# FabianPlum/SMILify

Measured on AMD Instinct MI355X. Metric: SMIL fit-iters/sec (LBS+render+loss) per GPU at 1/2/4/8 MI355X, higher is better.
Workload: dtype f32

## Files before the change

smilify_amd/csrc/raster.hip:

```cpp
#include "common.h"

#define TILE 8
#define DCHUNK 32
#define FREC 28
#define FSTR 28
#define K_EPS 1e-8f
#define ALPHA_GRAD_EPS 1e-12f
#ifndef SEL_BITS
#define SEL_BITS 5
#endif
#ifndef SEL1_BITS
#define SEL1_BITS 6
#endif
#define SAT8 160u
#ifndef DGROUP
#define DGROUP 4
#endif
#ifndef KGROUP
#define KGROUP 4
#endif
#ifndef SELR
#define SELR 6
#endif
#ifndef REC_CAP
#define REC_CAP 65536
#endif
#define REC_PAD 64
#ifndef RESIDENT_PER_CU
#define RESIDENT_PER_CU 16
#endif

#ifndef WAVES_PER_SIMD
#define WAVES_PER_SIMD 4
#endif
enum { MODE_FWD = 0, MODE_BWD = 1, MODE_FUSED = 2 };

#include "raster_hooks.h"

#define N_CLASSES 4
#ifndef PACKED_MIN_IMAGES
#define PACKED_MIN_IMAGES 64
#endif
#ifndef CLASS_T0
#define CLASS_T0 65536
#endif
#define CLASS_T1 16384
#define CLASS_T2 4096
#ifndef SPLIT0_LOG
#define SPLIT0_LOG 0
#endif
#define COUNT_TILES_MAX 4096
#define N_PARTS 8
struct RasterCounters {
    unsigned int n_class[N_PARTS][N_CLASSES];
    struct { unsigned int next, pad[15]; } deal[N_PARTS];
    unsigned int straddling;
    unsigned int unclipped;
    unsigned int tie_pixels;
    unsigned int tie_next;
};

__host__ __device__ __forceinline__ unsigned int deal_split_log(unsigned int n_items, unsigned int slots) {
    return n_items * 8u <= slots * 5u / 8u ? 3u : (n_items * 4u <= slots * 5u / 4u ? 2u : (n_items * 2u <= slots * 5u / 4u ? 1u : 0u));
}
__host__ __device__ __forceinline__ unsigned int deal_working(unsigned int n_items, unsigned int split_log, unsigned int slots) {
    const unsigned int w = (n_items << split_log) * 7u / 16u;
    return w > slots / 8u ? w : slots / 8u;
}

struct Rec3 { uint32_t a, b, c; };
struct TriIds { int a, b, c; };

#define CLIP_CUTS 1024
#define CLIP_FX (2 * CLIP_CUTS)
#define CLIP_VX (2 * CLIP_CUTS)
struct ClipTables {
    float *xv;
    int *xf;
    int2 *xsrc;
    float2 *xcoef;
    float *xg;
    uint32_t *xcount;
    int *xparent;
};
__host__ __device__ __forceinline__ int faces_padded(int F) { return (F + WAVE - 1) / WAVE * WAVE; }
__device__ __forceinline__ int face_vertex(const int *__restrict__ faces, const int *__restrict__ xf_n, int F, int f, int k) {
    return f < F ? faces[3 * f + k] : xf_n[3 * (f - faces_padded(F)) + k];
}
__device__ __forceinline__ const float *vertex_ptr(const float *__restrict__ vn, const float *__restrict__ xv_n, int V, int i) {
    return i < V ? vn + 3 * i : xv_n + 3 * (i - V);
}

struct RasterArgs {
    const float *verts_ndc;
    const int *faces;
    const uint32_t *tbox;
    const uint32_t *gbox;
    const uint4 *items;
    uint32_t item_cap;
    const float2 *fzr;
    RasterCounters *ctr;
    int N, V, F, S, tiles_x, K;
    int FT;
    ClipTables clip;
    float blur, sqrt_blur, inv_sigma, inv_sigma_log2e;
    float *sil;
    const float *grad_sil;
    const float *target;
    const uint8_t *target_u8;
    const float *pix_scale;
    const float *img_bound;
    int packed;
    float *loss_img;
    unsigned long long *loss_acc;
    float *d_ndc;
    const uint2 *lists;
    uint32_t list_cap;
    uint2 *slist;
    uint32_t *slist2;
    uint32_t *scfirst;
    float2 *sxy;
    TriIds *sid;
    Rec3 *srec;
    Rec3 *crec;
    int list_stride, n_cf;
    unsigned int slots;
    SmilClipDepth cd;
    int image0;
    int tie_rule;
    unsigned long long *tie_mask;
    HOOK_ARGS_FIELDS
};

__device__ __forceinline__ float pix_to_ndc(int i, int S) { return -1.0f + (2.0f * (float)i + 1.0f) / (float)S; }

__device__ __forceinline__ float edge_fn(float px, float py, float ax, float ay, float bx, float by) {
    return (px - ax) * (by - ay) - (py - ay) * (bx - ax);
}

__device__ __forceinline__ float image_fx_scale(float img_bound, float pix_scale, float inv_sigma) {
    const float bound = img_bound * fabsf(pix_scale) * sqrtf(inv_sigma);
    return (bound > 0.f && bound < 3.0e38f) ? exp2f(fminf(29.0f - floorf(log2f(bound)), 100.0f)) : 0.f;
}

template <typename T>
__device__ __forceinline__ uint32_t byte_offset(uint32_t i) {
    if (sizeof(T) == 12) {
        uint32_t r;
        asm("v_mul_u32_u24 %0, %1, 12" : "=v"(r) : "v"(i));
        return r;
    }
    return i * (uint32_t)sizeof(T);
}
template <typename T>
__device__ __forceinline__ T &at(T *base, uint32_t i) {
    i = HOOK_WRAP_IDX(i);
    return *reinterpret_cast<T *>(reinterpret_cast<char *>(base) + byte_offset<T>(i));
}
template <typename T>
__device__ __forceinline__ const T &at(const T *base, uint32_t i) {
    i = HOOK_WRAP_IDX(i);
    return *reinterpret_cast<const T *>(reinterpret_cast<const char *>(base) + byte_offset<T>(i));
}

__device__ __forceinline__ int wave_scan_add(int x) {
#define SCAN_STEP(ctrl, rows) { x += __builtin_amdgcn_update_dpp(0, x, ctrl, rows, 0xF, false); }
    SCAN_STEP(0x111, 0xF) SCAN_STEP(0x112, 0xF) SCAN_STEP(0x114, 0xF) SCAN_STEP(0x118, 0xF)
    SCAN_STEP(0x142, 0xA) SCAN_STEP(0x143, 0xC)
#undef SCAN_STEP
    return x;
}

#ifndef SETUP_THREADS
#define SETUP_THREADS 1024
#endif
// ... 697 lines not shown
    for (int i_ = lane; i_ < (1 << SEL_BITS) / 2 * WAVE; i_ += WAVE) lds.hist[i_] = 0u;
    __syncthreads();
    auto load_keys = [&](uint32_t (&kk)[KGROUP], uint32_t (&mt)[KGROUP], int g0) {
#pragma unroll
        for (int u = 0; u < KGROUP; ++u) {
            const uint32_t idx = (uint32_t)min(g0 + u * WAVE + lane, n_rec - 1);
            mt[u] = at(crec, idx).b;
            kk[u] = key_of(idx, mt[u]);
        }
    };
    auto count_keys = [&](const uint32_t (&kk)[KGROUP], const uint32_t (&mt)[KGROUP], int g0) {
        uint2 ps[KGROUP];
#pragma unroll
        for (int u = 0; u < KGROUP; ++u) ps[u] = lds.psel[mt[u] & 63u];
#pragma unroll
        for (int u = 0; u < KGROUP; ++u) {
            const uint32_t pxl = mt[u] & 63u;
            const bool hit = (g0 + u * WAVE + lane < n_rec) & (ps[u].y > 0u) & ((kk[u] >> nbits) == ps[u].x) & (kk[u] != 0xFFFFFFFFu);
            const uint32_t bucket = (kk[u] >> shift) & ((1u << b) - 1u);
            if (hit) atomicAdd(&lds.hist[(bucket >> 1) * WAVE + pxl], (bucket & 1u) ? 0x10000u : 1u);
        }
    };
    if (n_rec > 0) {
        uint32_t ka[KGROUP], ma[KGROUP], kb[KGROUP], mb[KGROUP];
        load_keys(ka, ma, 0);
        for (int g0 = 0; g0 < n_rec; g0 += 2 * KGROUP * WAVE) {
            load_keys(kb, mb, g0 + KGROUP * WAVE);
            count_keys(ka, ma, g0);
            load_keys(ka, ma, g0 + 2 * KGROUP * WAVE);
            count_keys(kb, mb, g0 + KGROUP * WAVE);
        }
    }
    __syncthreads();
}

__device__ __forceinline__ int refine_sweep(DenseLds &lds, Rec3 *crec, int n_rec, int nbits, int b,
                                            int lane, uint32_t pre, int need) {
    const int shift = nbits - b;
    lds.psel[lane] = make_uint2(pre, (uint32_t)need);
    for (int i_ = lane; i_ < (1 << SEL_BITS) / 2 * WAVE; i_ += WAVE) lds.hist[i_] = 0u;
    __syncthreads();
    int n_out = 0;
    struct CRec { uint32_t kk, mt; float lf; };
    auto load_recs = [&](CRec (&r)[KGROUP], int g0) {
#pragma unroll
        for (int u = 0; u < KGROUP; ++u) {
            const uint32_t idx = (uint32_t)min(g0 + u * WAVE + lane, n_rec - 1);
            const Rec3 q = at(crec, idx);
            r[u].kk = q.a; r[u].mt = q.b; r[u].lf = __uint_as_float(q.c);
        }
    };
    auto sift_recs = [&](const CRec (&r)[KGROUP], int g0) {
        uint2 ps[KGROUP];
#pragma unroll
        for (int u = 0; u < KGROUP; ++u) ps[u] = lds.psel[r[u].mt & 63u];
#pragma unroll
        for (int u = 0; u < KGROUP; ++u) {
            const uint32_t pxl = r[u].mt & 63u;
            const bool live = (g0 + u * WAVE + lane < n_rec) & (ps[u].y > 0u);
            const uint32_t top = r[u].kk >> nbits;
            const bool sure = live & (top < ps[u].x), stay = live & (top == ps[u].x);
            if (sure & (r[u].lf != 0.f)) atomicAdd(&lds.plog[pxl], (double)r[u].lf);
            const unsigned long long sm = __ballot(stay);
            const uint32_t slot = (uint32_t)n_out + __builtin_amdgcn_mbcnt_hi((uint32_t)(sm >> 32), __builtin_amdgcn_mbcnt_lo((uint32_t)sm, 0u));
            if (stay) {
                at(crec, slot) = Rec3{r[u].kk, r[u].mt, __float_as_uint(r[u].lf)};
                const uint32_t bucket = (r[u].kk >> shift) & ((1u << b) - 1u);
                atomicAdd(&lds.hist[(bucket >> 1) * WAVE + pxl], (bucket & 1u) ? 0x10000u : 1u);
            }
            n_out += __popcll(sm);
        }
    };
    if (n_rec > 0) {
        CRec ra[KGROUP], rb[KGROUP];
        load_recs(ra, 0);
        for (int g0 = 0; g0 < n_rec; g0 += 2 * KGROUP * WAVE) {
            load_recs(rb, g0 + KGROUP * WAVE);
            sift_recs(ra, g0);
            load_recs(ra, g0 + 2 * KGROUP * WAVE);
            sift_recs(rb, g0 + KGROUP * WAVE);
        }
    }
    __syncthreads();
    return n_out;
}

template <int MODE>
__global__ void __launch_bounds__(64, WAVES_PER_SIMD) k_raster_dense(RasterArgs a) {
    __shared__ DenseLds lds;
    const int lane = threadIdx.x;
    uint2 *const slist = a.slist + (size_t)blockIdx.x * a.list_stride;
    uint32_t *const slist2 = a.slist2 + (size_t)blockIdx.x * a.list_stride;
    uint32_t *const scfirst = a.scfirst + (size_t)blockIdx.x * a.n_cf;
    float2 *const sxy = a.sxy + (size_t)blockIdx.x * 3 * a.list_stride;
    TriIds *const sid = a.sid + (size_t)blockIdx.x * a.list_stride;
    const size_t rec0 = (size_t)blockIdx.x * (REC_CAP + REC_PAD);
    Rec3 *const srec = a.srec + rec0, *const crec = a.crec + rec0;
    const uint32_t lane_lo = lane < 32 ? 1u << lane : 0u, lane_hi = lane >= 32 ? 1u << (lane - 32) : 0u;
    const int K = a.K;
    const int n_tiles = a.tiles_x * a.tiles_x;
    unsigned int n_items_all = 0;
    for (int q = 0; q < N_PARTS; ++q)
        for (int c = 0; c < N_CLASSES; ++c) n_items_all += a.ctr->n_class[q][c];
    const unsigned int slots = a.slots;
    const unsigned int split_log = HOOK_SPLIT_LOG(deal_split_log(n_items_all, slots));
    if (blockIdx.x >= deal_working(n_items_all, split_log, slots)) return;
    const unsigned int split0_log = SPLIT0_LOG > split_log ? SPLIT0_LOG : split_log;
    const float fS = (float)a.S;
    unsigned int xcc;
    asm volatile("s_getreg_b32 %0, hwreg(HW_REG_XCC_ID)" : "=s"(xcc));
    xcc &= (unsigned int)(N_PARTS - 1);

    TIMERS_INIT
    for (unsigned int turn = 0; turn < N_PARTS; ++turn) {
    const unsigned int part = (xcc + turn) & (unsigned int)(N_PARTS - 1);
    const unsigned int nc0 = a.ctr->n_class[part][0], nc1 = a.ctr->n_class[part][1], nc2 = a.ctr->n_class[part][2], nc3 = a.ctr->n_class[part][3];
    const unsigned int n_items = nc0 + nc1 + nc2 + nc3;
    const unsigned int units0 = nc0 << split0_log;
    const unsigned int n_units = units0 + ((n_items - nc0) << split_log);
    const uint4 *const items = a.items + (size_t)part * 2u * a.item_cap;
    while (n_units > 0u) {
        unsigned int unit = 0;
        TSUB(0)
        if (lane == 0) unit = atomicAdd(&a.ctr->deal[part].next, 1u);
        unit = __builtin_amdgcn_readfirstlane(unit);
        if (unit >= n_units) break;
        TUNIT_START
        const bool heavy = unit < units0;
        const unsigned int sl = heavy ? split0_log : split_log, u_ = heavy ? unit : unit - units0;
        const unsigned int item = (u_ >> sl) + (heavy ? 0u : nc0);
        const int p_begin = (int)(u_ & ((1u << sl) - 1u)) * (WAVE >> sl), p_end = p_begin + (WAVE >> sl);
        const uint32_t item_at = item < nc0 ? item
                               : item < nc0 + nc1 ? a.item_cap - 1u - (item - nc0)
                               : item < nc0 + nc1 + nc2 ? a.item_cap + (item - nc0 - nc1)
                               : 2u * a.item_cap - 1u - (item - nc0 - nc1 - nc2);
        const uint4 it = items[item_at];
        const uint32_t code = it.x;
        const int n = (int)(code / (uint32_t)n_tiles), tile = (int)(code % (uint32_t)n_tiles);
        const int tx = tile % a.tiles_x, ty = tile / a.tiles_x;
        const int xo = tx * TILE + (lane & 7), yo = ty * TILE + (lane >> 3);
        const bool in_img = xo < a.S && yo < a.S;
        const float cx = pix_to_ndc(a.S - 1 - (tx * TILE + 4), a.S), cy = pix_to_ndc(a.S - 1 - (ty * TILE + 4), a.S);
        const float *vn = a.verts_ndc + (size_t)n * a.V * 3;
        const float *const xv_n = a.clip.xv + (size_t)n * CLIP_VX * 3;
        const int *const xf_n = a.clip.xf + (size_t)n * CLIP_FX * 3;
        const size_t pix = ((size_t)n * a.S + yo) * a.S + xo;

        uint32_t kmin, kmax;
        const uint2 td = make_uint2(it.y, it.z);
        const bool binned = td.y != 0xFFFFFFFFu;
        TSUB(1)
        const uint2 *const list_src = binned ? a.lists + (size_t)n * a.list_cap + td.x : slist;
        int list_total;
        if (binned) {
            list_total = (int)td.y;
            uint32_t lo = 0x7F7FFFFFu, hi = 0u;
            for (int i0 = 0; i0 < list_total; i0 += 4 * WAVE) {
                uint2 e[4];
#pragma unroll
                for (int u = 0; u < 4; ++u) e[u] = at(list_src, (uint32_t)min(i0 + u * WAVE + lane, list_total - 1));
#pragma unroll
                for (int u = 0; u < 4; ++u) { lo = min(lo, e[u].y); hi = max(hi, e[u].y); }
            }
            for (int o = 32; o > 0; o >>= 1) {
                lo = min(lo, (uint32_t)__shfl_xor((int)lo, o, WAVE));
                hi = max(hi, (uint32_t)__shfl_xor((int)hi, o, WAVE));
            }
            kmin = lo;
            kmax = __float_as_uint((__uint_as_float(hi) + __uint_as_float(it.w) * 1.000001f) * 1.0000005f) + 1u;
        } else {
            list_total = build_list(a, n, tx, ty, slist, lane, kmin, kmax);
        }
        const bool may_truncate = list_total > K;
        TSUB(2)
        const uint32_t krange = kmax - kmin;
        const int nbits0 = krange ? 32 - __clz(krange) : 0;
        const int b1 = min(SEL1_BITS, nbits0), shift1 = nbits0 - b1;
        __syncthreads();
        const uint32_t *const lst = slist2;
        if (may_truncate) {
            sort_list_near_to_far(list_src, slist2, list_total, kmin, shift1, b1, lds, lane);
        } else {
            for (int i = lane; i < list_total; i += WAVE) slist2[i] = at(list_src, (uint32_t)i).x;
            __syncthreads();
        }
        TMARK(0)
        TSUB(3)
        HOOK_STOP_AFTER(0, continue)

        unsigned long long tie_acc = 0ull;
        int span = p_end - p_begin;
        while (span > 1 && (long long)span * list_total > 4ll * REC_CAP) span >>= 1;
        for (int p_lo = p_begin; p_lo < p_end;) {
            const bool mine = lane >= p_lo && lane < p_lo + span;
            const int sy0 = p_lo >> 3, sy1 = (p_lo + span - 1) >> 3;
            const int sx0 = span >= 8 ? 0 : (p_lo & 7), sx1 = span >= 8 ? 7 : ((p_lo & 7) + span - 1);
            const float px = (in_img && mine) ? pix_to_ndc(a.S - 1 - xo, a.S) : 3.0e38f, py = pix_to_ndc(a.S - 1 - yo, a.S);
            lds.pixt[lane] = make_float2(px, py);
            if (may_truncate)
                for (int i_ = lane; i_ < (1 << SEL_BITS) / 2 * WAVE; i_ += WAVE) lds.hist[i_] = 0u;
            __syncthreads();

            int vbase = 0;
            bool fits = true;
            int final_digits = 0, final_cnt = 0;
            unsigned long long open_px = __ballot(in_img && mine);
            int ox0 = sx0, ox1 = sx1, oy0 = sy0, oy1 = sy1;
            int chunks_done = 0;
            uint32_t cst0 = 0u, cst1 = 0u;
            auto set_chunk_start = [&](int c, uint32_t v) {
                if (c < WAVE) cst0 = lane == c ? v : cst0;
                else if (c < 2 * WAVE) cst1 = lane == c - WAVE ? v : cst1;
                else if (lane == 0) scfirst[c] = v;
            };
            auto chunk_start = [&](int c) -> uint32_t {
                if (c < WAVE) return (uint32_t)__builtin_amdgcn_readlane((int)cst0, c);
                if (c < 2 * WAVE) return (uint32_t)__builtin_amdgcn_readlane((int)cst1, c - WAVE);
                return (uint32_t)__builtin_amdgcn_readfirstlane((int)scfirst[c]);
            };
            const int slot_ = lane & (DCHUNK - 1);
            auto list_at = [&](int c) { return (int)lst[min(c + slot_, list_total - 1)]; };
            int f_nx = list_at(2 * DCHUNK);
            int ia, ib, ic;
            int ja, jb, jc;
            Tri9 tv_nx;
            { const int f_ = list_at(0); ja = face_vertex(a.faces, xf_n, a.F, f_, 0); jb = face_vertex(a.faces, xf_n, a.F, f_, 1); jc = face_vertex(a.faces, xf_n, a.F, f_, 2); }
            { const int f_ = list_at(DCHUNK); ia = face_vertex(a.faces, xf_n, a.F, f_, 0); ib = face_vertex(a.faces, xf_n, a.F, f_, 1); ic = face_vertex(a.faces, xf_n, a.F, f_, 2); }
            tv_nx = load_tri(a, vn, xv_n, ja, jb, jc);
            for (int c0 = 0; c0 < list_total; c0 += DCHUNK) {
                if (may_truncate) {
                    const int d0 = __popcll(__ballot(lane < (1 << b1) && (int)lds.bstart[lane] <= c0)) - 1;
                    if (d0 > final_digits) {
                        for (int d = final_digits; d < d0; ++d)
                            final_cnt += (int)((lds.hist[(d >> 2) * WAVE + lane] >> (8 * (d & 3))) & 0xFFu);
                        final_digits = d0;
                        open_px &= ~__ballot(final_cnt >= K);
                        if (open_px == 0ull) break;
                        unsigned int cols = 0u;
                        oy0 = 8; oy1 = -1;
                        for (int y = 0; y < TILE; ++y) {
                            const unsigned int row = (unsigned int)(open_px >> (8 * y)) & 0xFFu;
                            cols |= row;
                            if (row) { oy0 = min(oy0, y); oy1 = y; }
                        }
                        ox0 = (int)__builtin_ctz(cols); ox1 = 31 - (int)__builtin_clz(cols);
                    }
                }
                const int m = min(DCHUNK, list_total - c0);
                int cf, packed2, packed = 0;
                const int i0 = ja, i1 = jb, i2 = jc;
                const Tri9 tv = tv_nx;
                ja = ia; jb = ib; jc = ic;
                tv_nx = load_tri(a, vn, xv_n, ja, jb, jc);
                ia = face_vertex(a.faces, xf_n, a.F, f_nx, 0); ib = face_vertex(a.faces, xf_n, a.F, f_nx, 1); ic = face_vertex(a.faces, xf_n, a.F, f_nx, 2);
                f_nx = list_at(c0 + 3 * DCHUNK);
                stage_faces(a, tv, i0, i1, i2, m, lds.rec, lane, cx, cy, fS, tx, ty, ox0, ox1, oy0, oy1, open_px, cf, packed2, sxy, sid, c0, a.list_stride);
                set_chunk_start(c0 / DCHUNK, (uint32_t)vbase);
                chunks_done = c0 / DCHUNK + 1;
                lds_fence();
                HOOK_STOP_AFTER(1, continue)
                const int incl = wave_scan_add(cf);
                const int off = incl - cf;
                const int n_pairs = __builtin_amdgcn_readlane(incl, 63);
                packed |= off;
                if (vbase + 2 * n_pairs > REC_CAP) { fits = false; break; }
                STAT(20, 2 * n_pairs)
                const unsigned long long nonempty = __ballot(cf > 0);
                STAT(31, __popcll(nonempty))
                lds.start[lane] = 0;
                lds_fence();
                if (cf > 0) {
                    atomicOr(reinterpret_cast<uint32_t *>(lds.start) + (off >> 5), 1u << (off & 31));
                    const uint32_t rank = __builtin_amdgcn_mbcnt_hi((uint32_t)(nonempty >> 32), __builtin_amdgcn_mbcnt_lo((uint32_t)nonempty, 0u));
                    lds.psel[rank] = make_uint2((uint32_t)packed | ((uint32_t)lane << 13), (uint32_t)packed2);
                }
                lds_fence();
                const uint32_t fl_lo = reinterpret_cast<const uint32_t *>(lds.start)[(2 * lane) & 63];
                const uint32_t fl_hi = reinterpret_cast<const uint32_t *>(lds.start)[(2 * lane + 1) & 63];
                const uint2 pk_rank = lds.psel[lane & (DCHUNK - 1)];
                lds_fence();
                TSTAGE_MARK
                uint32_t carry = 0;
                for (int q0 = 0; q0 < n_pairs; q0 += WAVE) {
                    const uint32_t wlo = (uint32_t)__builtin_amdgcn_readlane((int)fl_lo, q0 >> 6), whi = (uint32_t)__builtin_amdgcn_readlane((int)fl_hi, q0 >> 6);
                    const uint32_t below = __builtin_amdgcn_mbcnt_hi(whi, __builtin_amdgcn_mbcnt_lo(wlo, 0u));
                    const uint32_t own = ((wlo & lane_lo) | (whi & lane_hi)) ? 1u : 0u;
                    const int r = min((int)(carry + below + own) - 1, DCHUNK - 1);
                    carry += (uint32_t)(__popc(wlo) + __popc(whi));
                    const bool valid = q0 + lane < n_pairs;
                    const uint32_t pk = (uint32_t)__shfl((int)pk_rank.x, max(r, 0), WAVE), pk2 = (uint32_t)__shfl((int)pk_rank.y, max(r, 0), WAVE);
                    const int fs = (int)((pk >> 13) & (DCHUNK - 1));
                    const uint32_t rr = (uint32_t)(q0 + lane) - (pk & 0x1FFFu);
                    uint32_t rr_inv;
                    asm("v_mul_u32_u24 %0, %1, %2" : "=v"(rr_inv) : "v"(rr), "v"(pk2 & 0x1FFFFu));
                    const uint32_t dy = rr_inv >> 16;
                    const int pp = (int)((__umul24(dy, (pk2 >> 17) & 3u) + rr + (pk2 >> 20)) & 31u);
                    const int p = 2 * pp;
                    const float4 pc = *reinterpret_cast<const float4 *>(&lds.pixt[p]);
                    const FaceRows fr = load_face_rows(lds.rec + fs * FSTR);
                    PairEval2 e;
                    eval_pair2(fr, pc.x - cx, pc.z - cx, pc.y - cy, a.blur, e);
                    HOOK_EXTRA_VALU(pc)
                    const uint32_t open2 = (uint32_t)(open_px >> p) & 3u;
                    const bool cand0 = valid && e.cand0 && (open2 & 1u), cand1 = valid && e.cand1 && (open2 & 2u);
                    const unsigned long long cm0 = __ballot(cand0), cm1 = __ballot(cand1);
                    if ((cm0 | cm1) == 0ull) continue;
                    uint32_t zb0 = 0x7F61B1E6u, zb1 = 0x7F61B1E6u;
                    if (may_truncate) {
                        const f32x2 z2 = pair_depth2(fr, e);
                        const float zf = fminf(fminf(fr.r2.y, fr.r2.z), fr.r2.w);
                        zb0 = min(max(__float_as_uint(vmax_raw(z2.x, zf)), kmin), kmax);
                        zb1 = min(max(__float_as_uint(vmax_raw(z2.y, zf)), kmin), kmax);
                    }
                    const uint32_t slot0 = (uint32_t)vbase + __builtin_amdgcn_mbcnt_hi((uint32_t)(cm0 >> 32), __builtin_amdgcn_mbcnt_lo((uint32_t)cm0, 0u));
                    const uint32_t slot1 = (uint32_t)vbase + (uint32_t)__popcll(cm0) + __builtin_amdgcn_mbcnt_hi((uint32_t)(cm1 >> 32), __builtin_amdgcn_mbcnt_lo((uint32_t)cm1, 0u));
                    const uint32_t meta = (uint32_t)p | ((uint32_t)(c0 + fs) << 6);
                    if (cand0) {
                        st_stream(srec, slot0, Rec3{zb0, meta | (e.inside0 ? 1u << 22 : 0u) | e.ebits0, __float_as_uint(e.sd.x)});
                        if (may_truncate) {
                            const uint32_t bucket = ((zb0 - kmin) >> shift1) & ((1u << b1) - 1u);
                            uint32_t *const hw = &lds.hist[(bucket >> 2) * WAVE + p];
                            const uint32_t sh = 8u * (bucket & 3u);
                            if (((*hw >> sh) & 0xFFu) < SAT8) atomicAdd(hw, 1u << sh);
                        }
                    }
                    if (cand1) {
                        st_stream(srec, slot1, Rec3{zb1, (meta + 1u) | (e.inside1 ? 1u << 22 : 0u) | e.ebits1, __float_as_uint(e.sd.y)});
                        if (may_truncate) {
                            const uint32_t bucket = ((zb1 - kmin) >> shift1) & ((1u << b1) - 1u);
                            uint32_t *const hw = &lds.hist[(bucket >> 2) * WAVE + p + 1];
                            const uint32_t sh = 8u * (bucket & 3u);
                            if (((*hw >> sh) & 0xFFu) < SAT8) atomicAdd(hw, 1u << sh);
                        }
                    }
                    vbase += __popcll(cm0) + __popcll(cm1);
                }
                TSWEEP_MARK
                lds_fence();
            }
            if (!fits) {
                span >>= 1;
                __syncthreads();
                continue;
            }
            set_chunk_start(chunks_done, (uint32_t)vbase);
            STAT(21, vbase) STAT(26, 1) STAT(27, list_total) STAT(28, chunks_done) STAT(29, (list_total + DCHUNK - 1) / DCHUNK) STAT(30, __popcll(open_px))
            __syncthreads();
            TMARK(1)
            HOOK_STOP_AFTER(1, { p_lo += span; continue; }) HOOK_STOP_AFTER(2, { p_lo += span; continue; })

            uint32_t zt_bits = 0x7F800000u;
            int tie_cut = 0x7FFFFFFF;
            uint32_t pre = 0u;
            int need = 0, n_eq = 0, nbits = nbits0 - b1;
            bool trunc = false;
            bool defer = false;
            if (may_truncate && vbase > 0) {
                need = K;
                const int tot = pick_digit8(lds.hist, lane, b1, pre, need, n_eq);
                trunc = tot > K;
                if (!trunc) need = 0;
            }
            const bool any_trunc = __ballot(trunc) != 0ull;
            lds.plog[lane] = 0.0;
            lds.psel[lane] = make_uint2(pre, (uint32_t)need);
            const int b2 = min(SEL_BITS, nbits), shift2 = nbits - b2;
            if (any_trunc)
                for (int i_ = lane; i_ < (1 << SEL_BITS) / 2 * WAVE; i_ += WAVE) lds.hist[i_] = 0u;
            __syncthreads();
            TSUB(0)
            int n_cmp = 0;
            float rmax2 = 0.f;
            if (vbase > 0) {
                struct Rec { uint32_t z, mt; float sd; };
                auto load_recs = [&](Rec (&r)[DGROUP], int g0) {
#pragma unroll
                    for (int u = 0; u < DGROUP; ++u) {
                        const uint32_t idx = (uint32_t)min(g0 + u * WAVE + lane, vbase - 1);
                        const Rec3 q = ld_stream(srec, idx);
                        r[u].z = q.a; r[u].mt = q.b; r[u].sd = __uint_as_float(q.c);
                    }
                };
                auto blend_recs = [&](const Rec (&r)[DGROUP], int g0) {
                    uint2 ps[DGROUP];
#pragma unroll
                    for (int u = 0; u < DGROUP; ++u) ps[u] = lds.psel[r[u].mt & 63u];
#pragma unroll
                    for (int u = 0; u < DGROUP; ++u) {
                        const bool valid = g0 + u * WAVE + lane < vbase;
                        const uint32_t key = r[u].z - kmin, d1 = key >> nbits;
                        const bool sure = valid & ((ps[u].y == 0u) | (d1 < ps[u].x));
                        const bool maybe = valid & (ps[u].y > 0u) & (d1 == ps[u].x);
                        rmax2 = fmaxf(rmax2, fabsf(r[u].sd));
                        const float lf = __log2f(1.0f - face_prob(r[u].sd, a.inv_sigma_log2e));
                        if (sure & (lf != 0.f)) atomicAdd(&lds.plog[r[u].mt & 63u], (double)lf);
                        STAT(45, __popcll(__ballot(sure))) STAT(46, __popcll(__ballot(valid & !sure & !maybe)))
                        if (any_trunc) {
                            const unsigned long long km = __ballot(maybe);
                            const uint32_t slot = (uint32_t)n_cmp + __builtin_amdgcn_mbcnt_hi((uint32_t)(km >> 32), __builtin_amdgcn_mbcnt_lo((uint32_t)km, 0u));
                            if (maybe) {
                                at(crec, slot) = Rec3{key, r[u].mt, __float_as_uint(lf)};
                                const uint32_t bucket = (key >> shift2) & ((1u << b2) - 1u);
                                atomicAdd(&lds.hist[(bucket >> 1) * WAVE + (r[u].mt & 63u)], (bucket & 1u) ? 0x10000u : 1u);
                            }
                            n_cmp += __popcll(km);
                        }
                    }
                };
                Rec ra[DGROUP], rb[DGROUP];
                load_recs(ra, 0);
                for (int g0 = 0; g0 < vbase; g0 += 2 * DGROUP * WAVE) {
                    load_recs(rb, g0 + DGROUP * WAVE);
                    blend_recs(ra, g0);
                    load_recs(ra, g0 + 2 * DGROUP * WAVE);
                    blend_recs(rb, g0 + DGROUP * WAVE);
                }
            }
            __syncthreads();
            TSUB(4)
            if (any_trunc) {
                if (nbits > 0) {
                    pick_digit(lds.hist, lane, b2, pre, need, n_eq);
                    nbits -= b2;
                    __syncthreads();
                }
                while (nbits > 0 && __ballot(need > 0) != 0ull && n_cmp > SELR * WAVE) {
                    const int b = min(SEL_BITS, nbits);
                    n_cmp = refine_sweep(lds, crec, n_cmp, nbits, b, lane, pre, need);
                    pick_digit(lds.hist, lane, b, pre, need, n_eq);
                    nbits -= b;
                    __syncthreads();
                }
                if (n_cmp <= SELR * WAVE) {
                constexpr uint32_t INV = 0xFFFFFFFFu;
                uint32_t rk[SELR], rm[SELR];
                float rl[SELR];
#pragma unroll
                for (int r_ = 0; r_ < SELR; ++r_) {
                    const int idx = r_ * WAVE + lane;
                    const Rec3 q = at(crec, (uint32_t)min(idx, max(n_cmp - 1, 0)));
                    rk[r_] = idx < n_cmp ? q.a : INV; rm[r_] = q.b; rl[r_] = __uint_as_float(q.c);
                }
                while (nbits > 0 && __ballot(need > 0) != 0ull) {
                    const int b = min(SEL_BITS, nbits), shift = nbits - b;
                    lds.psel[lane] = make_uint2(pre, (uint32_t)need);
                    for (int i_ = lane; i_ < (1 << SEL_BITS) / 2 * WAVE; i_ += WAVE) lds.hist[i_] = 0u;
                    lds_fence();
                    uint2 ps[SELR];
#pragma unroll
                    for (int r_ = 0; r_ < SELR; ++r_) ps[r_] = lds.psel[rm[r_] & 63u];
#pragma unroll
                    for (int r_ = 0; r_ < SELR; ++r_) {
                        const uint32_t pxl = rm[r_] & 63u;
                        const bool live = (rk[r_] != INV) & (ps[r_].y > 0u);
                        const uint32_t top = rk[r_] >> nbits;
                        const bool sure = live & (top < ps[r_].x), stay = live & (top == ps[r_].x);
                        if (sure & (rl[r_] != 0.f)) atomicAdd(&lds.plog[pxl], (double)rl[r_]);
                        if (stay) {
                            const uint32_t bucket = (rk[r_] >> shift) & ((1u << b) - 1u);
                            atomicAdd(&lds.hist[(bucket >> 1) * WAVE + pxl], (bucket & 1u) ? 0x10000u : 1u);
                        }
                        rk[r_] = (live & !stay) ? INV : rk[r_];
                    }
                    lds_fence();
                    pick_digit(lds.hist, lane, b, pre, need, n_eq);
                    nbits -= b;
                    lds_fence();
                }
                if (trunc) zt_bits = pre + kmin;
                bool same = false;
                if (HOOK_TIE_EQUIV && a.tie_rule && __ballot(trunc && need < n_eq) != 0ull) {
                    lds.psel[lane] = make_uint2((trunc && need < n_eq) ? pre : INV, 0u);
                    lds.hist[lane] = 0xFFFFFFFFu; lds.hist[WAVE + lane] = 0u;
                    lds.hist[2 * WAVE + lane] = 1u; lds.hist[3 * WAVE + lane] = 0u;
                    lds_fence();
#pragma unroll
                    for (int r_ = 0; r_ < SELR; ++r_) {
                        const uint32_t pxl = rm[r_] & 63u;
                        if (rk[r_] != INV && rk[r_] == lds.psel[pxl].x) {
                            const uint32_t lb = __float_as_uint(rl[r_]), ins = (rm[r_] >> 22) & 1u;
                            atomicMin(&lds.hist[pxl], lb); atomicMax(&lds.hist[WAVE + pxl], lb);
                            atomicAnd(&lds.hist[2 * WAVE + pxl], ins); atomicOr(&lds.hist[3 * WAVE + pxl], ins);
                        }
                    }
                    lds_fence();
                    same = lds.hist[lane] == lds.hist[WAVE + lane] && lds.hist[2 * WAVE + lane] == lds.hist[3 * WAVE + lane];
                    lds_fence();
                }
                const bool split = trunc && need < n_eq && (!a.tie_rule || same);
                defer = trunc && need < n_eq && a.tie_rule && !same;
                uint32_t rf[SELR];
#pragma unroll
                for (int r_ = 0; r_ < SELR; ++r_) rf[r_] = INV;
                if (__ballot(split) != 0ull) {
                    lds.psel[lane] = make_uint2(split ? pre : INV, 0u);
                    lds_fence();
#pragma unroll
                    for (int r_ = 0; r_ < SELR; ++r_)
                        if (rk[r_] != INV && rk[r_] == lds.psel[rm[r_] & 63u].x) rf[r_] = lst[(rm[r_] >> 6) & 0xFFFFu];
                    int pbits = 32 - __clz(max(a.FT - 1, 1));
                    uint32_t ppre = 0u;
                    int pneed = split ? need : 0, peq = 0;
                    lds_fence();
                    while (pbits > 0 && __ballot(pneed > 0) != 0ull) {
                        const int b = min(SEL_BITS, pbits), shift = pbits - b;
                        lds.psel[lane] = make_uint2(ppre, (uint32_t)pneed);
                        for (int i_ = lane; i_ < (1 << SEL_BITS) / 2 * WAVE; i_ += WAVE) lds.hist[i_] = 0u;
                        lds_fence();
#pragma unroll
                        for (int r_ = 0; r_ < SELR; ++r_) {
                            const uint32_t pxl = rm[r_] & 63u;
                            const uint2 ps = lds.psel[pxl];
                            const bool hit = (rf[r_] != INV) & (ps.y > 0u) & ((rf[r_] >> pbits) == ps.x);
                            const uint32_t bucket = (rf[r_] >> shift) & ((1u << b) - 1u);
                            if (hit) atomicAdd(&lds.hist[(bucket >> 1) * WAVE + pxl], (bucket & 1u) ? 0x10000u : 1u);
                        }
                        lds_fence();
                        pick_digit(lds.hist, lane, b, ppre, pneed, peq);
                        pbits -= b;
                        lds_fence();
                    }
                    if (split) tie_cut = (int)ppre;
                }
                lds.psel[lane] = make_uint2(trunc ? pre : 0u, (uint32_t)tie_cut);
                lds_fence();
#pragma unroll
                for (int r_ = 0; r_ < SELR; ++r_) {
                    const uint32_t pxl = rm[r_] & 63u;
                    const uint2 ps = lds.psel[pxl];
                    const bool keep = (rk[r_] != INV) & ((rk[r_] < ps.x) | ((rk[r_] == ps.x) & (((int)ps.y == 0x7FFFFFFF) | ((int)rf[r_] <= (int)ps.y))));
                    if (keep & (rl[r_] != 0.f)) atomicAdd(&lds.plog[pxl], (double)rl[r_]);
                }
                lds_fence();
                } else {
                while (nbits > 0 && __ballot(need > 0) != 0ull) {
                    const int b = min(SEL_BITS, nbits);
                    n_cmp = refine_sweep(lds, crec, n_cmp, nbits, b, lane, pre, need);
                    pick_digit(lds.hist, lane, b, pre, need, n_eq);
                    nbits -= b;
                    __syncthreads();
                }
                if (trunc) zt_bits = pre + kmin;
                const bool split = trunc && need < n_eq && !a.tie_rule;
                defer = trunc && need < n_eq && a.tie_rule;
                if (__ballot(split) != 0ull) {
                    lds.pgrad[lane] = make_float4(0.f, __uint_as_float(split ? pre : 0xFFFFFFFFu), 0.f, 0.f);
                    __syncthreads();
                    int pbits = 32 - __clz(max(a.FT - 1, 1));
                    uint32_t ppre = 0u;
                    int pneed = split ? need : 0, peq = 0;
                    auto pos_key = [&](uint32_t idx, uint32_t mt) {
                        return at(crec, idx).a == __float_as_uint(lds.pgrad[mt & 63u].y) ? lst[(mt >> 6) & 0xFFFFu] : 0xFFFFFFFFu;
                    };
                    while (pbits > 0 && __ballot(pneed > 0) != 0ull) {
                        const int b = min(SEL_BITS, pbits);
                        select_sweep(lds, crec, n_cmp, pbits, b, lane, ppre, pneed, pos_key);
                        pick_digit(lds.hist, lane, b, ppre, pneed, peq);
                        pbits -= b;
                        __syncthreads();
                    }
                    if (split) tie_cut = (int)ppre;
                }
                lds.pgrad[lane] = make_float4(0.f, __uint_as_float(trunc ? pre : 0u), __int_as_float(tie_cut), 0.f);
                const bool any_split_sel = __ballot(tie_cut != 0x7FFFFFFF) != 0ull;
                __syncthreads();
                for (int g0 = 0; g0 < n_cmp; g0 += DGROUP * WAVE) {
                    uint32_t kk[DGROUP], mt[DGROUP];
                    float lf[DGROUP];
#pragma unroll
                    for (int u = 0; u < DGROUP; ++u) {
                        const uint32_t idx = (uint32_t)min(g0 + u * WAVE + lane, n_cmp - 1);
                        const Rec3 q = at(crec, idx);
                        kk[u] = q.a; mt[u] = q.b; lf[u] = __uint_as_float(q.c);
                    }
#pragma unroll
                    for (int u = 0; u < DGROUP; ++u) {
                        const float4 pg = lds.pgrad[mt[u] & 63u];
                        const uint32_t zt_ = __float_as_uint(pg.y);
                        const bool in_range = g0 + u * WAVE + lane < n_cmp;
                        bool tie_ok = true;
                        if (any_split_sel) {
                            const int cut = __float_as_int(pg.z);
                            int fid = 0;
                            if (in_range & (kk[u] == zt_) & (cut != 0x7FFFFFFF)) fid = (int)lst[(mt[u] >> 6) & 0xFFFFu];
                            tie_ok = fid <= cut;
                        }
                        const bool keep = in_range & ((kk[u] < zt_) | ((kk[u] == zt_) & tie_ok));
                        if (keep & (lf[u] != 0.f)) atomicAdd(&lds.plog[mt[u] & 63u], (double)lf[u]);
                    }
                }
                __syncthreads();
                }
            }
            TMARK(2)
            TSUB(5)
            HOOK_STOP_AFTER(3, { p_lo += span; continue; })
            STAT(22, n_cmp) STAT(23, __popcll(__ballot(trunc))) STAT(24, __popcll(__ballot(lds.plog[lane] != 0.0)))
            STAT(40, any_trunc ? 1 : 0) STAT(41, may_truncate ? 1 : 0) STAT(42, any_trunc ? vbase : 0) STAT(43, may_truncate ? vbase : 0) STAT(44, __popcll(__ballot(tie_cut != 0x7FFFFFFF)))
            const double plog_px = lds.plog[lane];
            const float alpha = exp2f((float)plog_px);
            TMARK(3)

            const float silv = 1.0f - alpha;
            const bool own = in_img && mine && !defer;
            tie_acc |= __ballot(in_img && mine && defer);
            float g = 0.f;
            if (MODE == MODE_FWD) {
                if (own) a.sil[pix] = silv;
            } else if (MODE == MODE_BWD) {
                if (own) g = a.grad_sil[pix];
            } else {
                float lsum = 0.f;
                if (own) {
                    const float tg = a.target_u8 ? (float)a.target_u8[pix] : a.target[pix];
                    const float diff = silv - tg;
                    lsum = fabsf(diff) - fabsf(tg);
                    g = a.pix_scale[n] * (diff > 0.f ? 1.f : (diff < 0.f ? -1.f : 0.f));
                    if (a.sil) a.sil[pix] = silv;
                }
                lsum = wave_sum(lsum);
                if (lane == 0 && lsum != 0.f) atomicAdd(&a.loss_acc[n], (unsigned long long)(long long)rint((double)lsum * 4294967296.0));
            }

            const float coef = -g * alpha * a.inv_sigma;
            const bool active = own && (g != 0.f) && (alpha > ALPHA_GRAD_EPS) && (plog_px != 0.0);
            const bool any_split = __ballot(tie_cut != 0x7FFFFFFF) != 0ull;
            TSUB(6)
            STAT(25, __popcll(__ballot(active)))
            if (MODE != MODE_FWD && __ballot(active) != 0ull) {
                float *dn = a.d_ndc + (size_t)n * a.V * 2;
                const float csum = wave_sum(active ? fabsf(coef) : 0.f);
                const float bound = 2.0f * sqrtf(wave_max(rmax2)) * csum;
                const bool img_fixed = MODE == MODE_FUSED && a.packed && a.clip.xcount[n] == 0u;
                const float fx_scale = img_fixed ? image_fx_scale(a.img_bound[n], a.pix_scale[n], a.inv_sigma)
                                       : (bound > 0.f && bound < 3.0e38f) ? exp2f(fminf(29.0f - floorf(log2f(bound)), 100.0f)) : 0.f;
                const float fx_inv = fx_scale > 0.f ? 1.0f / fx_scale : 0.f;
                lds.pgrad[lane] = make_float4(active ? coef * fx_scale : 0.f, __uint_as_float(zt_bits), __int_as_float(tie_cut), 0.f);
                __syncthreads();
                constexpr int GR = GCHUNK / DCHUNK;
                static_assert(GCHUNK == WAVE, "pass 3: lane = face of the group");
                const uint32_t copy_off = (uint32_t)(lane & (GCOPIES - 1)) * (GCHUNK * 3);
                float *const xg_n = a.clip.xg + (size_t)n * CLIP_VX * 2;
                float2 *const fv = reinterpret_cast<float2 *>(lds.hist);
                static_assert(GCHUNK * 3 * sizeof(float2) <= sizeof(lds.hist), "the vertex table of a group lives in the histogram area");
                TP3_START
                for (int ch = 0; ch < chunks_done; ch += GR) {
                    const int i_beg = (int)chunk_start(ch), i_end = (int)chunk_start(min(ch + GR, chunks_done));
                    if (i_beg == i_end) continue;
                    TP3(0)
                    const int fch = ch * DCHUNK + lane;
                    const bool staged = fch < chunks_done * DCHUNK && fch < list_total;
                    const uint32_t fcl = (uint32_t)min(fch, list_total - 1);
                    const float2 tv0 = at(sxy, fcl), tv1 = at(sxy, (uint32_t)a.list_stride + fcl), tv2 = at(sxy, 2u * (uint32_t)a.list_stride + fcl);
                    const TriIds tid = at(sid, fcl);
                    struct GRec { uint32_t z, mt; float sd; };
                    auto load_recs = [&](GRec (&r)[DGROUP], int g0) {
#pragma unroll
                        for (int u = 0; u < DGROUP; ++u) {
                            const uint32_t idx = (uint32_t)min(g0 + u * WAVE + lane, i_end - 1);
                            const Rec3 q = ld_stream(srec, idx);
                            r[u].z = q.a; r[u].mt = q.b; r[u].sd = __uint_as_float(q.c);
                        }
                    };
                    GRec ra[DGROUP], rb[DGROUP];
                    load_recs(ra, i_beg);
                    fv[lane * 3 + 0] = tv0;
                    fv[lane * 3 + 1] = tv1;
                    fv[lane * 3 + 2] = tv2;
                    TP3(1)
                    for (int i_ = lane; i_ < GCOPIES * GCHUNK * 3; i_ += WAVE) (&lds.gacc[0][0])[i_] = 0ull;
                    lds_fence();
                    TP3(2)
                    auto grad_recs = [&](const GRec (&r)[DGROUP], int g0) {
                        float4 pg[DGROUP];
                        float2 pa[DGROUP], pb[DGROUP], pc[DGROUP];
                        uint32_t oa[DGROUP], ob[DGROUP];
#pragma unroll
                        for (int u = 0; u < DGROUP; ++u) {
                            const uint32_t mt = r[u].mt;
                            const uint32_t f3 = ((mt >> 6) & (uint32_t)(GCHUNK - 1)) * 3u;
                            const uint32_t edge = mt >> 23;
                            oa[u] = f3 + (edge == 2u ? 1u : 0u); ob[u] = f3 + (edge == 0u ? 1u : 2u);
                            pg[u] = lds.pgrad[mt & 63u];
                            pa[u] = fv[oa[u]]; pb[u] = fv[ob[u]]; pc[u] = lds.pixt[mt & 63u];
                        }
#pragma unroll
                        for (int u = 0; u < DGROUP; ++u) {
                            const bool valid = g0 + u * WAVE + lane < i_end;
                            const uint32_t mt = r[u].mt;
                            const uint32_t zt_ = __float_as_uint(pg[u].y);
                            const bool inside = ((mt >> 22) & 1u) != 0u;
                            float gd = pg[u].x * face_prob(r[u].sd, a.inv_sigma_log2e);
                            gd = inside ? -gd : gd;
                            bool tie_ok = true;
                            if (any_split) {
                                const int cut = __float_as_int(pg[u].z);
                                int fid = 0;
                                if (valid & (r[u].z == zt_) & (cut != 0x7FFFFFFF)) fid = (int)lst[(mt >> 6) & 0xFFFFu];
                                tie_ok = fid <= cut;
                            }
                            const bool keep = valid & (gd != 0.f) & ((r[u].z < zt_) | ((r[u].z == zt_) & tie_ok));
                            const float exx = pb[u].x - pa[u].x, eyy = pb[u].y - pa[u].y;
                            const float l2 = exx * exx + eyy * eyy;
                            const float t = __builtin_amdgcn_fmed3f((exx * (pc[u].x - pa[u].x) + eyy * (pc[u].y - pa[u].y)) * (l2 <= K_EPS ? 0.f : __builtin_amdgcn_rcpf(l2)), 0.f, 1.f);
                            const float rx = fmaf(t, exx, pa[u].x - pc[u].x), ry = fmaf(t, eyy, pa[u].y - pc[u].y);
                            const float ex = 2.0f * rx * gd, ey = 2.0f * ry * gd;
                            const float bx = t * ex, by = t * ey;
                            auto pack = [](float x, float y) {
                                const int qx = cvt_round(x), qy = cvt_round(y);
                                return ((unsigned long long)(uint32_t)(qx + (qy >> 31)) << 32) | (unsigned long long)(uint32_t)qy;
                            };
                            const unsigned long long ga = pack(ex - bx, ey - by), gb = pack(bx, by);
                            if (keep) {
                                unsigned long long *acc = &lds.gacc[0][0] + copy_off;
                                atomicAdd(acc + oa[u], ga);
                                atomicAdd(acc + ob[u], gb);
                            }
                        }
                    };
                    for (int g0 = i_beg; g0 < i_end; g0 += 2 * DGROUP * WAVE) {
                        load_recs(rb, g0 + DGROUP * WAVE);
                        grad_recs(ra, g0);
                        load_recs(ra, g0 + 2 * DGROUP * WAVE);
                        grad_recs(rb, g0 + DGROUP * WAVE);
                    }
                    TP3(3)
                    lds_fence();
                    TP3(4)
                    if (staged) {
                        const int vi[3] = {tid.a, tid.b, tid.c};
#pragma unroll
                        for (int k = 0; k < 3; ++k) {
                            unsigned long long tot = 0ull;
#pragma unroll
                            for (int c = 0; c < GCOPIES; ++c) tot += lds.gacc[c][lane * 3 + k];
                            if (img_fixed) {
                                if (tot != 0ull) atomicAdd(reinterpret_cast<unsigned long long *>(dn) + vi[k], tot);
                                continue;
                            }
                            const int qy = (int)(uint32_t)tot;
                            const int qx = (int)(uint32_t)((tot - (unsigned long long)(long long)qy) >> 32);
                            float *const row = vi[k] < a.V ? dn + 2 * vi[k] : xg_n + 2 * (vi[k] - a.V);
                            if (qx != 0) atomicAdd(row, (float)qx * fx_inv);
                            if (qy != 0) atomicAdd(row + 1, (float)qy * fx_inv);
                        }
                    }
                    lds_fence();
                    TP3(5)
                }
            }
            __syncthreads();
            TMARK(4)
            TSUB(7)
            p_lo += span;
        }
        if (tie_acc != 0ull && lane == 0) {
            atomicOr(&a.tie_mask[(size_t)part * 2u * a.item_cap + item_at], tie_acc);
            atomicAdd(&a.ctr->tie_pixels, (unsigned int)__popcll(tie_acc));
        }
        TUNIT_END
    }
    }
    TIMERS_FLUSH
}

__device__ __forceinline__ FaceRows face_rows_from_tri(const Tri9 &tv, float cx, float cy) {
    FaceRows q;
    float rl12;
    face_rows_lo(tv, cx, cy, q.r0, q.r1, q.r2);
    face_rows_hi(tv, cx, cy, q.r3, q.r4, q.r5, rl12);
    q.r6 = make_float4(rl12, 0.f, 0.f, 0.f);
    return q;
}
__device__ __forceinline__ uint32_t wave_max_u32(uint32_t v) {
    int x = (int)v;
#define MAX_STEP(ctrl, rows) { x = (int)max((uint32_t)x, (uint32_t)__builtin_amdgcn_update_dpp(0, x, ctrl, rows, 0xF, false)); }
    MAX_STEP(0x111, 0xF) MAX_STEP(0x112, 0xF) MAX_STEP(0x114, 0xF) MAX_STEP(0x118, 0xF)
    MAX_STEP(0x142, 0xA) MAX_STEP(0x143, 0xC)
#undef MAX_STEP
    return (uint32_t)__builtin_amdgcn_readlane(x, WAVE - 1);
}
__device__ __forceinline__ double wave_sum_f64(double v) {
    for (int o = 32; o > 0; o >>= 1) v += __shfl_xor(v, o, WAVE);
    return v;
}

#ifndef TIE_WHOLE_TILE
#define TIE_WHOLE_TILE 6
#endif
#ifndef TIE_ORD_CAP
#define TIE_ORD_CAP 2048
#endif
static_assert(TIE_ORD_CAP % 64 == 0 && TIE_ORD_CAP / 32 <= WAVE && TIE_ORD_CAP >= 64 * 32, "the high bits of the ordered ids are cleared by one wave; a segment of 64 bitmap words fits");
#ifndef TIE_WAVES_PER_SIMD
#define TIE_WAVES_PER_SIMD 5
#endif
template <int MODE>
__global__ void __launch_bounds__(64, TIE_WAVES_PER_SIMD) k_raster_tie_replay(RasterArgs a) {
    const int lane = threadIdx.x;
    const int K = a.K;
    const int n_tiles = a.tiles_x * a.tiles_x;
    const int n_groups = a.FT / WAVE;
    extern __shared__ uint32_t tie_lds[];
    uint32_t *const bm = tie_lds;
    uint32_t *const fz = tie_lds + a.FT / 32, *const fm = fz + 2 * WAVE;
    float *const fs = reinterpret_cast<float *>(fm + 2 * WAVE);
    uint16_t *const ord = reinterpret_cast<uint16_t *>(fm + 4 * WAVE);
    uint32_t *const ord_hi = fm + 4 * WAVE + TIE_ORD_CAP / 2;
    const int bm_words = a.FT / 32;
    unsigned int total = 0;
    for (int q = 0; q < N_PARTS; ++q)
        for (int c = 0; c < N_CLASSES; ++c) total += a.ctr->n_class[q][c];
    unsigned int pre[N_PARTS + 1];
    pre[0] = 0u;
    for (int q = 0; q < N_PARTS; ++q) pre[q + 1] = pre[q] + a.ctr->n_class[q][0] + a.ctr->n_class[q][1] + a.ctr->n_class[q][2] + a.ctr->n_class[q][3];
    if (blockIdx.x >= a.ctr->tie_pixels) return;
    const unsigned int px_per_wave = a.ctr->tie_pixels / gridDim.x;
    unsigned int parts_log = px_per_wave >= 16u ? 2u : (px_per_wave >= 4u ? 4u : 6u);
    while (((unsigned long long)total << parts_log) > 0xFFFFFFC0ull) --parts_log;
    const unsigned int px_log = 6u - parts_log;
    const unsigned int n_units = total << parts_log, n_tickets = (n_units + (unsigned int)WAVE - 1u) / (unsigned int)WAVE;
    TIE_TIMERS_INIT
    for (;;) {
        TIE_T(5)
        unsigned int ticket = 0u;
        if (lane == 0) ticket = atomicAdd(&a.ctr->tie_next, 1u);
        ticket = (unsigned int)__builtin_amdgcn_readfirstlane((int)ticket);
        if (ticket >= n_tickets) break;
        TIE_T(4)
        const unsigned int u = (unsigned int)lane * n_tickets + ticket;
        unsigned long long my_mask = 0ull;
        uint32_t my_slot = 0u;
        if (u < n_units) {
            const unsigned int quarter = u / total, idx = u - quarter * total;
            int part = 0;
#pragma unroll
            for (int q = 1; q < N_PARTS; ++q) part += idx >= pre[q] ? 1 : 0;
            const unsigned int item = idx - pre[part];
            const unsigned int nc0 = a.ctr->n_class[part][0], nc1 = a.ctr->n_class[part][1], nc2 = a.ctr->n_class[part][2];
            const uint32_t item_at = item < nc0 ? item
                                   : item < nc0 + nc1 ? a.item_cap - 1u - (item - nc0)
                                   : item < nc0 + nc1 + nc2 ? a.item_cap + (item - nc0 - nc1)
                                   : 2u * a.item_cap - 1u - (item - nc0 - nc1 - nc2);
            my_slot = (uint32_t)part * 2u * a.item_cap + item_at;
            const unsigned long long full = a.tie_mask[my_slot];
            const unsigned long long part_mask = ((px_log == 6u ? 0ull : 1ull << (1u << px_log)) - 1ull) << (quarter << px_log);
            my_mask = (parts_log == 2u && __popcll(full) <= TIE_WHOLE_TILE) ? (quarter == 0u ? full : 0ull) : full & part_mask;
        }
        unsigned long long um = __ballot(my_mask != 0ull);
        TIE_T(4)
        while (um) {
        const int ul = (int)__builtin_ctzll(um);
        um &= um - 1ull;
        const size_t slot_i = (size_t)(uint32_t)__builtin_amdgcn_readlane((int)my_slot, ul);
        unsigned long long mask = (unsigned long long)(uint32_t)__builtin_amdgcn_readlane((int)(uint32_t)my_mask, ul) |
                                  ((unsigned long long)(uint32_t)__builtin_amdgcn_readlane((int)(uint32_t)(my_mask >> 32), ul) << 32);
        const uint4 it = a.items[slot_i];
        const uint32_t code = it.x;
        const int n = (int)(code / (uint32_t)n_tiles), tile = (int)(code % (uint32_t)n_tiles);
        const int tx = tile % a.tiles_x, ty = tile / a.tiles_x;
        const float cx = pix_to_ndc(a.S - 1 - (tx * TILE + 4), a.S), cy = pix_to_ndc(a.S - 1 - (ty * TILE + 4), a.S);
        const float *vn = a.verts_ndc + (size_t)n * a.V * 3;
        const float *const xv_n = a.clip.xv + (size_t)n * CLIP_VX * 3;
        const int *const xf_n = a.clip.xf + (size_t)n * CLIP_FX * 3;
        const uint32_t *__restrict__ tbox_n = a.tbox + (size_t)n * a.FT;
        const uint32_t *__restrict__ gbox_n = a.gbox + (size_t)n * n_groups;
        const float2 *__restrict__ fzr_n = a.fzr + (size_t)n * a.FT;
        __syncthreads();
        for (int w = lane; w < bm_words; w += WAVE) bm[w] = 0u;
        __syncthreads();
        if (it.z != 0xFFFFFFFFu) {
            const uint2 *const ls = a.lists + (size_t)n * a.list_cap + it.y;
            for (int i = lane; i < (int)it.z; i += WAVE) {
                const uint32_t f = ls[i].x;
                atomicOr(&bm[f >> 5], 1u << (f & 31u));
            }
        } else {
            for (int g = 0; g < n_groups; ++g)
                if (box_has(gbox_n[g], tx, ty)) {
                    const unsigned long long hit = __ballot(box_has(tbox_n[g * WAVE + lane], tx, ty));
                    if (lane == 0) { bm[2 * g] = (uint32_t)hit; bm[2 * g + 1] = (uint32_t)(hit >> 32); }
                }
        }
        __syncthreads();
        auto extract = [&](int w0, int w1) -> int {
            int cnt = 0;
            if (lane < TIE_ORD_CAP / 32) ord_hi[lane] = 0u;
            __syncthreads();
            for (int wb = w0; wb < w1; wb += WAVE) {
                uint32_t wv = wb + lane < w1 ? bm[wb + lane] : 0u;
                const int c = __popc(wv), inc = wave_scan_add(c);
                int o = cnt + inc - c;
                while (wv) {
                    const uint32_t id = (uint32_t)((wb + lane) * 32 + (__ffs((int)wv) - 1));
                    ord[o] = (uint16_t)id;
                    if (id >> 16) atomicOr(&ord_hi[o >> 5], 1u << (o & 31));
                    ++o;
                    wv &= wv - 1u;
                }
                cnt += __builtin_amdgcn_readlane(inc, WAVE - 1);
            }
            __syncthreads();
            return cnt;
        };
        int n_faces = 0;
        for (int w = lane; w < bm_words; w += WAVE) n_faces += __popc(bm[w]);
        n_faces = __builtin_amdgcn_readlane(wave_scan_add(n_faces), WAVE - 1);
// ... 474 lines not shown
```

Baseline: 75.37.

## Stage short binned face lists in LDS and bucket-sort them in place

For binned tiles whose list fits in LIST_LDS_ROWS*WAVE entries, the kernel now copies the list from global memory into the record/histogram LDS region once, while it computes the depth range. The near-to-far bucket sort then runs from LDS instead of re-reading global memory, and the first three chunks' face ids go into a small head buffer held in psel. The first vertex-id fetch is hoisted out of the sub-tile loop and reissued on each sub-tile advance or span halving. One __syncthreads is dropped on the LDS path, which relies on a single wave per block and lds_fence ordering. The change also hides the lane value behind an opaque asm to steer register allocation, and it aliases LDS regions, which risks clobbering data if the layout assumptions are wrong.

```diff
diff --git a/smilify_amd/csrc/raster.hip b/smilify_amd/csrc/raster.hip
--- a/smilify_amd/csrc/raster.hip
+++ b/smilify_amd/csrc/raster.hip
@@ -21,6 +21,9 @@
 #endif
 #ifndef SELR
 #define SELR 6
+#endif
+#ifndef LIST_LDS_ROWS
+#define LIST_LDS_ROWS 8
 #endif
 #ifndef REC_CAP
 #define REC_CAP 65536
@@ -1024,7 +1027,49 @@
         TSUB(1)
         const uint2 *const list_src = binned ? a.lists + (size_t)n * a.list_cap + td.x : slist;
         int list_total;
-        if (binned) {
+        const bool list_lds = LIST_LDS_ROWS > 0 && binned && td.y <= (uint32_t)(LIST_LDS_ROWS * WAVE);
+        uint2 *const llist = reinterpret_cast<uint2 *>(&lds);
+        static_assert(LIST_LDS_ROWS * WAVE * sizeof(uint2) <= offsetof(DenseLds, pixt), "the list lives in the record and histogram areas");
+        uint32_t *const head = reinterpret_cast<uint32_t *>(lds.psel);
+        static_assert(3 * DCHUNK * sizeof(uint32_t) <= sizeof(lds.psel), "the list's head lives in psel");
+        if (list_lds) {
+            list_total = (int)td.y;
+            kmin = 0u;
+            kmax = 0u;
+            if (list_total > K) {
+                uint32_t lo = 0x7F7FFFFFu, hi = 0u;
+                for (int i0 = 0; i0 < list_total; i0 += 4 * WAVE) {
+                    uint2 e[4];
+#pragma unroll
+                    for (int u = 0; u < 4; ++u) e[u] = at(list_src, (uint32_t)min(i0 + u * WAVE + lane, list_total - 1));
+#pragma unroll
+                    for (int u = 0; u < 4; ++u) {
+                        lo = min(lo, e[u].y); hi = max(hi, e[u].y);
+                        if (i0 + u * WAVE + lane < list_total) llist[i0 + u * WAVE + lane] = e[u];
+                    }
+                }
+                for (int o = 32; o > 0; o >>= 1) {
+                    lo = min(lo, (uint32_t)__shfl_xor((int)lo, o, WAVE));
+                    hi = max(hi, (uint32_t)__shfl_xor((int)hi, o, WAVE));
+                }
+                kmin = lo;
+                kmax = __float_as_uint((__uint_as_float(hi) + __uint_as_float(it.w) * 1.000001f) * 1.0000005f) + 1u;
+            } else {
+                for (int i0 = 0; i0 < list_total; i0 += 4 * WAVE) {
+                    uint2 e[4];
+#pragma unroll
+                    for (int u = 0; u < 4; ++u) e[u] = at(list_src, (uint32_t)min(i0 + u * WAVE + lane, list_total - 1));
+#pragma unroll
+                    for (int u = 0; u < 4; ++u) {
+                        const int pos = i0 + u * WAVE + lane;
+                        if (pos < list_total) {
+                            slist2[pos] = e[u].x;
+                            if (pos < 3 * DCHUNK) head[pos] = e[u].x;
+                        }
+                    }
+                }
+            }
+        } else if (binned) {
             list_total = (int)td.y;
             uint32_t lo = 0x7F7FFFFFu, hi = 0u;
             for (int i0 = 0; i0 < list_total; i0 += 4 * WAVE) {
@@ -1048,13 +1093,64 @@
         const uint32_t krange = kmax - kmin;
         const int nbits0 = krange ? 32 - __clz(krange) : 0;
         const int b1 = min(SEL1_BITS, nbits0), shift1 = nbits0 - b1;
-        __syncthreads();
         const uint32_t *const lst = slist2;
-        if (may_truncate) {
-            sort_list_near_to_far(list_src, slist2, list_total, kmin, shift1, b1, lds, lane);
+        const int slot_ = lane & (DCHUNK - 1);
+        auto list_at = [&](int c) { return (int)lst[min(c + slot_, list_total - 1)]; };
+        int f_nx;
+        int ia, ib, ic;
+        int ja, jb, jc;
+        auto fetch_ids = [&](int f0, int f1) {
+            ja = face_vertex(a.faces, xf_n, a.F, f0, 0); jb = face_vertex(a.faces, xf_n, a.F, f0, 1); jc = face_vertex(a.faces, xf_n, a.F, f0, 2);
+            ia = face_vertex(a.faces, xf_n, a.F, f1, 0); ib = face_vertex(a.faces, xf_n, a.F, f1, 1); ic = face_vertex(a.faces, xf_n, a.F, f1, 2);
+        };
+        auto first_ids = [&]() { f_nx = list_at(2 * DCHUNK); fetch_ids(list_at(0), list_at(DCHUNK)); };
+        if (list_lds) {
+            if (may_truncate) {
+                const int n_buckets = 1 << b1;
+                auto digit_of = [&](const uint2 &e) { return (int)(((e.y - kmin) >> shift1) & (uint32_t)(n_buckets - 1)); };
+                lds.start[lane] = 0;
+                lds_fence();
+                for (int i0 = 0; i0 < list_total; i0 += 4 * WAVE) {
+                    uint2 e[4];
+#pragma unroll
+                    for (int u = 0; u < 4; ++u) e[u] = llist[min(i0 + u * WAVE + lane, list_total - 1)];
+#pragma unroll
+                    for (int u = 0; u < 4; ++u)
+                        if (i0 + u * WAVE + lane < list_total) atomicAdd(&lds.start[digit_of(e[u])], 1);
+                }
+                lds_fence();
+                const int c = lane < n_buckets ? lds.start[lane] : 0;
+                const int incl = wave_scan_add(c);
+                lds_fence();
+                if (lane < n_buckets) lds.bstart[lane] = (uint16_t)min(incl - c, 65535);
+                lds.start[lane] = incl - c;
+                lds_fence();
+                for (int i0 = 0; i0 < list_total; i0 += 4 * WAVE) {
+                    uint2 e[4];
+#pragma unroll
+                    for (int u = 0; u < 4; ++u) e[u] = llist[min(i0 + u * WAVE + lane, list_total - 1)];
+#pragma unroll
+                    for (int u = 0; u < 4; ++u)
+                        if (i0 + u * WAVE + lane < list_total) {
+                            const int pos = atomicAdd(&lds.start[digit_of(e[u])], 1);
+                            slist2[pos] = e[u].x;
+                            if (pos < 3 * DCHUNK) head[pos] = e[u].x;
+                        }
+                }
+            }
+            lds_fence();
+            auto head_at = [&](int c) { return (int)head[min(c + slot_, list_total - 1)]; };
+            f_nx = head_at(2 * DCHUNK);
+            fetch_ids(head_at(0), head_at(DCHUNK));
         } else {
-            for (int i = lane; i < list_total; i += WAVE) slist2[i] = at(list_src, (uint32_t)i).x;
             __syncthreads();
+            if (may_truncate) {
+                sort_list_near_to_far(list_src, slist2, list_total, kmin, shift1, b1, lds, lane);
+            } else {
+                for (int i = lane; i < list_total; i += WAVE) slist2[i] = at(list_src, (uint32_t)i).x;
+                __syncthreads();
+            }
+            first_ids();
         }
         TMARK(0)
         TSUB(3)
@@ -1063,7 +1159,14 @@
         unsigned long long tie_acc = 0ull;
         int span = p_end - p_begin;
         while (span > 1 && (long long)span * list_total > 4ll * REC_CAP) span >>= 1;
-        for (int p_lo = p_begin; p_lo < p_end;) {
+        int p_lo = p_begin;
+        auto next_sub_tile = [&]() -> bool {
+            p_lo += span;
+            if (p_lo >= p_end) return false;
+            first_ids();
+            return true;
+        };
+        for (;;) {
             const bool mine = lane >= p_lo && lane < p_lo + span;
             const int sy0 = p_lo >> 3, sy1 = (p_lo + span - 1) >> 3;
             const int sx0 = span >= 8 ? 0 : (p_lo & 7), sx1 = span >= 8 ? 7 : ((p_lo & 7) + span - 1);
@@ -1090,14 +1193,7 @@
                 if (c < 2 * WAVE) return (uint32_t)__builtin_amdgcn_readlane((int)cst1, c - WAVE);
                 return (uint32_t)__builtin_amdgcn_readfirstlane((int)scfirst[c]);
             };
-            const int slot_ = lane & (DCHUNK - 1);
-            auto list_at = [&](int c) { return (int)lst[min(c + slot_, list_total - 1)]; };
-            int f_nx = list_at(2 * DCHUNK);
-            int ia, ib, ic;
-            int ja, jb, jc;
             Tri9 tv_nx;
-            { const int f_ = list_at(0); ja = face_vertex(a.faces, xf_n, a.F, f_, 0); jb = face_vertex(a.faces, xf_n, a.F, f_, 1); jc = face_vertex(a.faces, xf_n, a.F, f_, 2); }
-            { const int f_ = list_at(DCHUNK); ia = face_vertex(a.faces, xf_n, a.F, f_, 0); ib = face_vertex(a.faces, xf_n, a.F, f_, 1); ic = face_vertex(a.faces, xf_n, a.F, f_, 2); }
             tv_nx = load_tri(a, vn, xv_n, ja, jb, jc);
             for (int c0 = 0; c0 < list_total; c0 += DCHUNK) {
                 if (may_truncate) {
@@ -1120,13 +1216,15 @@
                 }
                 const int m = min(DCHUNK, list_total - c0);
                 int cf, packed2, packed = 0;
+                int lane_c = lane;
+                asm volatile("" : "+v"(lane_c));
                 const int i0 = ja, i1 = jb, i2 = jc;
                 const Tri9 tv = tv_nx;
                 ja = ia; jb = ib; jc = ic;
                 tv_nx = load_tri(a, vn, xv_n, ja, jb, jc);
                 ia = face_vertex(a.faces, xf_n, a.F, f_nx, 0); ib = face_vertex(a.faces, xf_n, a.F, f_nx, 1); ic = face_vertex(a.faces, xf_n, a.F, f_nx, 2);
                 f_nx = list_at(c0 + 3 * DCHUNK);
-                stage_faces(a, tv, i0, i1, i2, m, lds.rec, lane, cx, cy, fS, tx, ty, ox0, ox1, oy0, oy1, open_px, cf, packed2, sxy, sid, c0, a.list_stride);
+                stage_faces(a, tv, i0, i1, i2, m, lds.rec, lane_c, cx, cy, fS, tx, ty, ox0, ox1, oy0, oy1, open_px, cf, packed2, sxy, sid, c0, a.list_stride);
                 set_chunk_start(c0 / DCHUNK, (uint32_t)vbase);
                 chunks_done = c0 / DCHUNK + 1;
                 lds_fence();
@@ -1139,7 +1237,7 @@
                 STAT(20, 2 * n_pairs)
                 const unsigned long long nonempty = __ballot(cf > 0);
                 STAT(31, __popcll(nonempty))
-                lds.start[lane] = 0;
+                lds.start[lane_c] = 0;
                 lds_fence();
                 if (cf > 0) {
                     atomicOr(reinterpret_cast<uint32_t *>(lds.start) + (off >> 5), 1u << (off & 31));
@@ -1213,13 +1311,14 @@
             if (!fits) {
                 span >>= 1;
                 __syncthreads();
+                first_ids();
                 continue;
             }
             set_chunk_start(chunks_done, (uint32_t)vbase);
             STAT(21, vbase) STAT(26, 1) STAT(27, list_total) STAT(28, chunks_done) STAT(29, (list_total + DCHUNK - 1) / DCHUNK) STAT(30, __popcll(open_px))
             __syncthreads();
             TMARK(1)
-            HOOK_STOP_AFTER(1, { p_lo += span; continue; }) HOOK_STOP_AFTER(2, { p_lo += span; continue; })
+            HOOK_STOP_AFTER(1, { if (!next_sub_tile()) break; continue; }) HOOK_STOP_AFTER(2, { if (!next_sub_tile()) break; continue; })
 
             uint32_t zt_bits = 0x7F800000u;
             int tie_cut = 0x7FFFFFFF;
@@ -1466,7 +1565,7 @@
             }
             TMARK(2)
             TSUB(5)
-            HOOK_STOP_AFTER(3, { p_lo += span; continue; })
+            HOOK_STOP_AFTER(3, { if (!next_sub_tile()) break; continue; })
             STAT(22, n_cmp) STAT(23, __popcll(__ballot(trunc))) STAT(24, __popcll(__ballot(lds.plog[lane] != 0.0)))
             STAT(40, any_trunc ? 1 : 0) STAT(41, may_truncate ? 1 : 0) STAT(42, any_trunc ? vbase : 0) STAT(43, may_truncate ? vbase : 0) STAT(44, __popcll(__ballot(tie_cut != 0x7FFFFFFF)))
             const double plog_px = lds.plog[lane];
@@ -1624,7 +1723,7 @@
             __syncthreads();
             TMARK(4)
             TSUB(7)
-            p_lo += span;
+            if (!next_sub_tile()) break;
         }
         if (tie_acc != 0ull && lane == 0) {
             atomicOr(&a.tie_mask[(size_t)part * 2u * a.item_cap + item_at], tie_acc);
```

Result: faster. 76.34, median of 6 (+1.3%).
